# NVIDIA-Merlin/distributed-embeddings

Hardware: NVIDIA H100
Metric: DLRM global samples/sec (device-timed, max over ranks) (higher is better)
Workload: dtype bf16

## Files before the change

distributed_embeddings_b200/models/dlrm_fast.py:

```python
from __future__ import annotations

import os
from typing import Optional

import torch
from torch import nn

from ..ops import _native
from ..parallel.comm import CommContext
from ..parallel.fused import FusedEngine
from ..utils import nvtx
from ..utils.lr_schedule import LearningRateScheduler
from .dlrm import DLRM


def _pad8(n: int) -> int:
  return (n + 7) // 8 * 8


class _Layer:

  def __init__(self, lin: nn.Linear, relu: bool):
    self.lin = lin
    self.relu = relu
# ... 75 lines not shown
      dp_targets = []
      for layer, (off, shape) in zip(self.emb.dp_layers, self._dp_slots):
        n = shape[0] * shape[1]
        view = self.p32[off:off + n].view(shape)
        view.copy_(layer.embeddings.data)
        layer.embeddings.data = view
        dp_targets.append(self.g32[off:off + n].view(shape))
      if self._dp_slots:
        self.engine.set_dp_grad_targets(dp_targets)
        self.engine._tables_dirty = True
        self.engine._key = None
      for L in layers:
        wv = self.p32[L.w_off:L.w_off + L.w_numel].view(L.out_f, L.in_pad)
        wv[:, :L.in_f].copy_(L.lin.weight)
        L.lin.weight.data = wv[:, :L.in_f]
        bv = self.p32[L.b_off:L.b_off + L.out_f]
        bv.copy_(L.lin.bias)
        L.lin.bias.data = bv
        L.w16 = self.p16[L.w_off:L.w_off + L.w_numel].view(L.out_f, L.in_pad)
        L.b16 = self.p16[L.b_off:L.b_off + L.out_f]
        L.gw = self.g32[L.w_off:L.w_off + L.w_numel].view(L.out_f, L.in_pad)
        L.gb = self.g32[L.b_off:L.b_off + L.b_numel]
        L.w16T = torch.empty(L.in_pad, L.out_f, dtype=torch.bfloat16, device=dev)
      self.p16.copy_(self.p32)
      self._refresh_transposes()
    self.lr_t = torch.full((1,), float(lr), dtype=torch.float32, device=dev)
    self.engine.share_lr(self.lr_t)
    self.lr = float(lr)
    self.loss = torch.zeros(1, dtype=torch.float32, device=dev)
    self._batch = None
    self._graph = None
    self._side = torch.cuda.Stream(device=dev) if overlap else None
    self._wgrad_overlap = os.environ.get("DE_B200_WGRAD_STREAM", "auto")
    self._wstream = torch.cuda.Stream(device=dev) if overlap else None
    ar_env = os.environ.get("DE_B200_AR_OVERLAP", "auto")
    ar_on = ar_env == "1" or (ar_env == "auto" and self.world >= 4)
    self._ar_stream = torch.cuda.Stream(device=dev) if (overlap and self.world > 1 and ar_on) \
        else None

  def _refresh_transposes(self):
    if self.gemm == "cublas":
      return
    for L in self.bottom[1:] + self.top[1:]:
      L.w16T.copy_(L.w16.t())

  def _linear_fwd(self, L, x):
    if self.gemm in ("tcgen05", "tcgen05_pair"):
      pair = self.gemm == "tcgen05_pair" and L.out_f >= 256
      self.ops.gemm_tn_bias_act(x, L.w16, L.b16, L.y, True, 512 if pair else 0)
    else:
      torch._addmm_activation(L.b16, x, L.w16.t(), out=L.y)
    return L.y

  def _wgrad(self, L, x):
    use = self._wstream is not None and (
        self._wgrad_overlap == "1" or
        (self._wgrad_overlap == "auto" and (self._batch or 0) >= 49152))
    if not use:
      torch.mm(L.dy.t(), x, out_dtype=torch.float32, out=L.gw)
      return
    self._w_used = True
    self._wstream.wait_stream(torch.cuda.current_stream())
    with torch.cuda.stream(self._wstream):
      torch.mm(L.dy.t(), x, out_dtype=torch.float32, out=L.gw)

  def _dgrad_relu(self, L, x_below, dx, gb_below):
    if self.gemm == "cublas":
      torch.mm(L.dy, L.w16, out=dx)
      self.ops.relu_bwd_bias(dx, x_below, gb_below)
    else:
      self.ops.gemm_dgrad_relu_bias(L.dy, L.w16T, x_below, dx, gb_below, 0)

  def _alloc(self, b: int):
    dev, bf = self.dev, torch.bfloat16
    if self._stream_push:
      self.engine.enable_streamed_push(max(1024, -(-b // 16)))
    self.engine.prepare(b, [1] * self.n_emb, ids64=False)
    self.cat_stage = self.engine.in_flat[:self.n_emb * b].view(self.n_emb, b)
    self.num_in = torch.zeros(b, self.bottom[0].in_f, dtype=torch.float32, device=dev)
    self.lab_in = torch.zeros(b, dtype=torch.float32, device=dev)
    self.x0 = torch.zeros(b, self.bottom[0].in_pad, dtype=bf, device=dev)
    for L in self.bottom + self.top:
      L.y = torch.empty(b, L.out_f, dtype=bf, device=dev)
      L.dy = torch.empty(b, L.out_f, dtype=bf, device=dev)
    self.z = torch.zeros(b, self.top[0].in_pad, dtype=bf, device=dev)
    self.dz = torch.empty(b, self.top[0].in_pad, dtype=bf, device=dev)
    self._batch = b
    self._graph = None
    self._stage = [(torch.zeros_like(self.cat_stage), torch.zeros_like(self.num_in),
                    torch.zeros_like(self.lab_in)) for _ in range(2)]
    self._slot_dev = torch.zeros(1, dtype=torch.int32, device=dev)
    self._slot_host = torch.tensor([[0], [1]], dtype=torch.int32).pin_memory()
    self._h2d_done = [torch.cuda.Event(), torch.cuda.Event()]
    self._consumed = [torch.cuda.Event(), torch.cuda.Event()]
# ... 41 lines not shown
      L = self.top[i]
      x = self.top[i - 1].y if i > 0 else self.z
      dx = self.top[i - 1].dy if i > 0 else self.dz
      self._wgrad(L, x)
      if i > 0:
        self._dgrad_relu(L, x, dx, self.top[i - 1].gb)
      else:
        torch.mm(L.dy, L.w16, out=dx)
    if self._ar_stream is not None:
      ar = self._ar_stream
      ar.wait_stream(torch.cuda.current_stream())
      if getattr(self, "_w_used", False):
        ar.wait_stream(self._wstream)
      off = self.top[0].w_off
      with torch.cuda.stream(ar):
        self.ctx.allreduce_(self.gsym, self.n_flat - off, torch.float32, scale=1.0 / self.world,
                            byte_offset=off * 4, max_blocks=32)
    hb = self.bottom[-1]
    pushed = eng.streamed_push
    if pushed:
      eng.push_counters.zero_()
      self._push_ready.record(torch.cuda.current_stream())
      ops.interact_bwd(hb.y, eng.out, self.n_emb, self.dz, hb.dy, 0, 0, 1.0, eng.routes_stage,
                       len(eng.routes_stage_np), [], eng.push_counters, eng.push_chunk_rows)
      self._push_stream.wait_event(self._push_ready)
      with torch.cuda.stream(self._push_stream):
        eng.launch_streamed_push()
    else:
      ops.interact_bwd(hb.y, eng.out, self.n_emb, self.dz, hb.dy, 0, 0, 1.0, eng.routes_all,
                       len(eng.routes_all_np), eng.sync_grad_signal(), None, 0)
    if self._side is not None:
      self._side.wait_stream(torch.cuda.current_stream())
      if pushed:
        self._side.wait_stream(self._push_stream)
      with torch.cuda.stream(self._side):
        eng.backward_inplace()
    else:
      if pushed:
        torch.cuda.current_stream().wait_stream(self._push_stream)
      eng.backward_inplace()
    ops.relu_bwd_bias(hb.dy, hb.y, hb.gb)
    for i in range(len(self.bottom) - 1, -1, -1):
      L = self.bottom[i]
      x = self.bottom[i - 1].y if i > 0 else self.x0
      self._wgrad(L, x)
      if i > 0:
        self._dgrad_relu(L, x, self.bottom[i - 1].dy, self.bottom[i - 1].gb)
    if self._dp_slots and self._side is not None:
      torch.cuda.current_stream().wait_stream(self._side)
    if getattr(self, "_w_used", False):
      torch.cuda.current_stream().wait_stream(self._wstream)
      self._w_used = False
    if self.world > 1:
      if self._ar_stream is not None:
        ar = self._ar_stream
        ar.wait_stream(torch.cuda.current_stream())
        with torch.cuda.stream(ar):
          self.ctx.allreduce_(self.gsym, self.top[0].w_off, torch.float32, scale=1.0 / self.world)
        torch.cuda.current_stream().wait_stream(ar)
      else:
        self.ctx.allreduce_(self.gsym, self.n_flat, torch.float32, scale=1.0 / self.world)
    ops.dense_sgd(self.p32, self.p16, self.g32, self.lr_t, 1.0)
    self._refresh_transposes()
    if self._side is not None:
# ... 86 lines not shown
```

distributed_embeddings_b200/ops/csrc/bindings.cpp:

```cpp
#include <ATen/cuda/CUDAContext.h>
#include <c10/cuda/CUDAGuard.h>
#include <c10/cuda/CUDAStream.h>
#include <cuda_runtime.h>
#include <torch/library.h>
#include <torch/torch.h>

#include <cstdlib>
#include <cstring>
#include <mutex>
#include <string>
#include <unordered_map>
#include <vector>

#include "de_b200.h"

namespace {

using at::Tensor;

#define DE_CUDA_CHECK(expr)                                                              \
  do {                                                                                   \
    cudaError_t _e = (expr);                                                             \
    TORCH_CHECK(_e == cudaSuccess, "CUDA error in " #expr ": ", cudaGetErrorString(_e)); \
  } while (0)
// ... 696 lines not shown
}

void interact_fwd(const Tensor& bottom, const Tensor& emb, int64_t n_emb, Tensor z,
                  at::IntArrayRef sync) {
  check_bf16_2d(bottom, "bottom");
  check_bf16_2d(emb, "emb");
  check_bf16_2d(z, "z");
  c10::cuda::CUDAGuard guard(bottom.device());
  const int64_t dim = bottom.size(1);
  TORCH_CHECK(emb.size(1) == n_emb * dim);
  const int64_t need = (n_emb + 1) * n_emb / 2 + dim;
  TORCH_CHECK(z.size(1) >= need, "z is too narrow");
  bool ok = de::launch_interact_fwd(bottom.data_ptr(), bottom.stride(0), emb.data_ptr(),
                                    emb.stride(0), static_cast<int>(n_emb), static_cast<int>(dim),
                                    z.data_ptr(), z.stride(0), static_cast<int>(z.size(1)),
                                    bottom.size(0), sm_count(), cur_stream(), to_sync(sync));
  TORCH_CHECK(ok, "unsupported interaction shape (n_emb <= 31, dim in {16,32,64,128})");
  check_launch();
}

void interact_bwd(const Tensor& bottom, const Tensor& emb, int64_t n_emb, const Tensor& dz,
                  Tensor dbottom, int64_t demb_ptr, int64_t demb_stride, double emb_grad_scale,
                  const c10::optional<Tensor>& routes, int64_t n_routes, at::IntArrayRef sync,
                  const c10::optional<Tensor>& done_counters, int64_t chunk_rows) {
  check_bf16_2d(bottom, "bottom");
  check_bf16_2d(emb, "emb");
  check_bf16_2d(dz, "dz");
  check_bf16_2d(dbottom, "dbottom");
  if (routes.has_value())
    TORCH_CHECK(routes->is_cuda() && routes->scalar_type() == at::kByte &&
                routes->numel() >= n_routes * static_cast<int64_t>(sizeof(de::GradRoute)));
  c10::cuda::CUDAGuard guard(bottom.device());
  const int64_t dim = bottom.size(1);
  bool ok = de::launch_interact_bwd(bottom.data_ptr(), bottom.stride(0), emb.data_ptr(),
                                    emb.stride(0), static_cast<int>(n_emb), static_cast<int>(dim),
                                    dz.data_ptr(), dz.stride(0), dbottom.data_ptr(),
                                    dbottom.stride(0), reinterpret_cast<void*>(demb_ptr),
                                    demb_stride, static_cast<float>(emb_grad_scale),
                                    bottom.size(0), sm_count(), cur_stream(),
                                    routes.has_value()
                                        ? reinterpret_cast<const de::GradRoute*>(routes->data_ptr())
                                        : nullptr,
                                    static_cast<int>(n_routes), to_sync(sync),
                                    done_counters.has_value()
                                        ? reinterpret_cast<uint32_t*>(done_counters->data_ptr<int>())
                                        : nullptr,
                                    static_cast<int>(chunk_rows));
  TORCH_CHECK(ok, "unsupported interaction shape (n_emb <= 31, dim in {32,64,128}; routed / "
                  "signalling launches need dim in {64,128} and 16-byte aligned rows)");
  check_launch();
}

void avgpool_fwd(const Tensor& x, int64_t n, Tensor out, int64_t stride) {
  check_bf16_2d(x, "x");
  check_bf16_2d(out, "out");
  const int64_t out_len = (n + stride - 1) / stride;
  TORCH_CHECK(x.size(1) >= n && out.size(1) >= out_len && out.size(0) == x.size(0));
  const int64_t pad = std::max<int64_t>(0, (out_len - 1) * stride + stride - n);
  c10::cuda::CUDAGuard guard(x.device());
  de::launch_avgpool_fwd(x.data_ptr(), x.stride(0), static_cast<int>(n), out.data_ptr(),
                         out.stride(0), static_cast<int>(out_len), static_cast<int>(stride),
                         static_cast<int>(pad / 2), x.size(0), cur_stream());
  check_launch();
}

void avgpool_bwd(const Tensor& dout, Tensor dx, int64_t n, int64_t stride) {
  check_bf16_2d(dout, "dout");
  check_bf16_2d(dx, "dx");
  const int64_t out_len = (n + stride - 1) / stride;
  TORCH_CHECK(dx.size(1) >= n && dout.size(1) >= out_len && dout.size(0) == dx.size(0));
// ... 221 lines not shown
      "-> ()",
      &push_grad);
  m.def(
      "stream_push(int[] src_ptrs, int[] dst_ptrs, int[] row_bytes, Tensor counters, "
      "int chunk_rows, int rows, int blocks, int[] sync) -> ()",
      &stream_push);
  m.def(
      "rowslice_reduce(Tensor partial, int out_ptr, int out_stride, int out_dtype, Tensor cols) "
      "-> ()",
      &rowslice_reduce);
  m.def(
      "gather_ragged(Tensor segs, int[] val_ptrs, int[] split_ptrs, Tensor(a!) dst_vals, "
      "Tensor(b!) goff, int b, int max_cap) -> ()",
      &gather_ragged);
  m.def("select_copy(Tensor[] src0, Tensor[] src1, Tensor(a!)[] dst, Tensor slot_flag) -> ()",
        &select_copy);
  m.def("copy_cast_2d(Tensor src, int dst_ptr, int dst_stride, int dst_dtype, float scale) -> ()",
        &copy_cast_2d);
  m.def("interact_fwd(Tensor bottom, Tensor emb, int n_emb, Tensor(a!) z, int[] sync) -> ()",
        &interact_fwd);
  m.def(
      "interact_bwd(Tensor bottom, Tensor emb, int n_emb, Tensor dz, Tensor(a!) dbottom, "
      "int demb_ptr, int demb_stride, float emb_grad_scale, Tensor? routes, int n_routes, "
      "int[] sync, Tensor? done_counters, int chunk_rows) -> ()",
      &interact_bwd);
  m.def("avgpool_fwd(Tensor x, int n, Tensor(a!) out, int stride) -> ()", &avgpool_fwd);
  m.def("avgpool_bwd(Tensor dout, Tensor(a!) dx, int n, int stride) -> ()", &avgpool_bwd);
  m.def("relu_bwd_bias(Tensor(a!) dy, Tensor y, Tensor(b!) db) -> ()", &relu_bwd_bias);
  m.def(
      "head_loss(Tensor x, Tensor w, Tensor bias, Tensor labels, float inv_batch, Tensor(a!) dx, "
      "Tensor(b!) dw, Tensor(c!) db, Tensor(d!) dbias_prev, Tensor(e!) loss_sum, Tensor? logits) "
      "-> ()",
      &head_loss);
  m.def(
      "dense_sgd(Tensor(a!) p32, Tensor(b!) p16, Tensor(c!) g32, Tensor lr, float grad_scale) "
      "-> ()",
      &dense_sgd);
  m.def("cast_pad(Tensor src, Tensor(a!) dst) -> ()", &cast_pad);
  m.def(
      "gemm_tn_bias_act(Tensor a, Tensor b, Tensor? bias, Tensor(a!) out, bool relu, int block_n) "
      "-> ()",
      &gemm_tn_bias_act);
  m.def(
      "gemm_dgrad_relu_bias(Tensor dy, Tensor wt, Tensor act, Tensor(a!) dx, Tensor(b!) colsum, "
      "int block_n) -> ()",
      &gemm_dgrad_relu_bias);
  m.def("symm_alloc(int nbytes, int device_index) -> Tensor", &symm_alloc);
// ... 6 lines not shown
```

distributed_embeddings_b200/ops/csrc/de_b200.h:

```cpp
#pragma once
#include <cuda_runtime.h>
#include <stdint.h>

namespace de {

constexpr int kMaxPeers = 16;
constexpr int kGridCapSms = 132;

struct alignas(16) InputDesc {
  const void* table;
  const void* ids;
  const int64_t* offsets;
  int64_t ids_off;
  int64_t id_shift;
  int64_t sub_rows;
  int64_t row_base;
  int32_t width;
  int32_t hotness;
  int32_t dst_col;
  int32_t combiner;
  int32_t local_table;
  int32_t flags;
  int64_t item_off;
};
// ... 144 lines not shown
                            int n_cols, cudaStream_t stream);
void launch_gather_segments(const int64_t* segs, int n_seg, const PeerPtrs& src, void* dst,
                            int elem_bytes, int64_t max_seg_elems, cudaStream_t stream);
void launch_gather_ragged(const int64_t* segs, int n_seg, const PeerPtrs& src_vals,
                          const PeerPtrs& src_splits, void* dst_vals, int64_t* goff, int64_t b,
                          int world, int elem_bytes, int64_t max_cap, cudaStream_t stream);
void launch_select_copy(const void* const* src0, const void* const* src1, void* const* dst,
                        const int64_t* nbytes, int count, const int* slot_flag, int sm_count,
                        cudaStream_t stream);
void launch_copy_cast_2d(const void* src, int64_t src_stride, void* dst, int64_t dst_stride,
                         int64_t rows, int64_t cols, int src_dtype, int dst_dtype, float scale,
                         cudaStream_t stream);

bool launch_interact_fwd(const void* bottom, int64_t bottom_stride, const void* emb,
                         int64_t emb_stride, int n_emb, int dim, void* z, int64_t z_stride,
                         int z_width, int64_t batch, int sm_count, cudaStream_t stream,
                         const SyncArgs& sync);
bool launch_interact_bwd(const void* bottom, int64_t bottom_stride, const void* emb,
                         int64_t emb_stride, int n_emb, int dim, const void* dz,
                         int64_t dz_stride, void* dbottom, int64_t dbottom_stride, void* demb,
                         int64_t demb_stride, float emb_grad_scale, int64_t batch, int sm_count,
                         cudaStream_t stream, const GradRoute* routes, int n_routes,
                         const SyncArgs& sync, uint32_t* done_counters = nullptr,
                         int chunk_rows = 0);
void launch_avgpool_fwd(const void* x, int64_t x_stride, int n, void* out, int64_t out_stride,
                        int out_len, int stride, int left, int64_t rows, cudaStream_t stream);
void launch_avgpool_bwd(const void* dout, int64_t dout_stride, int out_len, void* dx,
                        int64_t dx_stride, int n, int stride, int left, int64_t rows,
                        cudaStream_t stream);
void launch_relu_bwd_bias(void* dy, const void* y, float* db, int64_t rows, int cols,
                          cudaStream_t stream);
bool launch_head_loss(const void* x, int K, const void* w, const void* bias, const float* labels,
                      int64_t batch, float inv_batch, void* dx, float* dw, float* db,
                      float* dbias_prev, float* loss_sum, float* logits_out, int sm_count,
                      cudaStream_t stream);
void launch_sgd_update(float* p32, void* p16, float* g32, const float* lr_ptr, float grad_scale,
                       int64_t n, int sm_count, cudaStream_t stream);
void launch_cast_pad(const float* src, int src_cols, void* dst, int dst_cols, int64_t rows,
                     cudaStream_t stream);

bool launch_gemm_tn_fused(const void* A, int64_t lda, const void* B, int64_t ldb, const void* bias,
                          void* C, int64_t ldc, int M, int N, int K, int epi, const void* act,
                          int64_t ldact, float* colsum, int block_n, int sm_count,
                          cudaStream_t stream);
bool launch_gemm_tn_bias_act(const void* A, int64_t lda, const void* B, int64_t ldb,
                             const void* bias, void* C, int64_t ldc, int M, int N, int K,
                             bool relu, int block_n, int sm_count, cudaStream_t stream);
// ... 3 lines not shown
```

distributed_embeddings_b200/ops/csrc/dense_kernels.cu:

```cuda
#include <cuda_bf16.h>
#include <cuda_runtime.h>
#include <stdint.h>

#include <cstdlib>

#include "common.cuh"
#include "de_b200.h"

namespace de {

namespace {

using bf16 = __nv_bfloat16;

__device__ __forceinline__ uint32_t smem_u32(const void* p) {
  return static_cast<uint32_t>(__cvta_generic_to_shared(p));
}

__device__ __forceinline__ void ldmatrix_x4(uint32_t (&r)[4], uint32_t addr) {
  asm volatile("ldmatrix.sync.aligned.m8n8.x4.shared.b16 {%0,%1,%2,%3}, [%4];"
               : "=r"(r[0]), "=r"(r[1]), "=r"(r[2]), "=r"(r[3])
               : "r"(addr));
}
__device__ __forceinline__ void ldmatrix_x4_trans(uint32_t (&r)[4], uint32_t addr) {
// ... 226 lines not shown
#pragma unroll 4
  for (int c = lane; c < total; c += 32) {
    const int row = c / kChunks, ch = c - row * kChunks;
    const bf16* src = row == 0 ? bottom + ch * 8 : emb + (row - 1) * D + ch * 8;
    cp_async16(sF + row * LD + ch * 8, src);
  }
  for (int c = lane; c < dz_chunks; c += 32) cp_async16(sDz + c * 8, dz + c * 8);
}

struct ChunkDst {
  unsigned long long base;
  long long stride;
};

template <int D>
__global__ void __launch_bounds__(kWarps * 32)
interact_bwd_v2_kernel(const bf16* __restrict__ bottom, int64_t bottom_stride,
                       const bf16* __restrict__ emb, int64_t emb_stride, int n_emb,
                       const bf16* __restrict__ dz, int64_t dz_stride, bf16* __restrict__ dbottom,
                       int64_t dbottom_stride, bf16* __restrict__ demb, int64_t demb_stride,
                       float emb_grad_scale, int64_t batch,
                       const GradRoute* __restrict__ routes, int n_routes,
                       const __grid_constant__ SyncArgs sync, uint32_t* __restrict__ done_counters,
                       int chunk_rows) {
  constexpr int LD = D + 8;
  constexpr int LDG = 40;
  constexpr int kWarpElems = 2 * kMaxFeat * LD + 2 * kDzMax + kMaxFeat * LDG;
  constexpr int kRowChunks = D / 8;
  extern __shared__ __align__(16) unsigned char smem_raw[];
  const int warp = threadIdx.x >> 5, lane = threadIdx.x & 31;
  bf16* base = reinterpret_cast<bf16*>(smem_raw) + warp * kWarpElems;
  bf16* sDz0 = base + 2 * kMaxFeat * LD;
  bf16* sG = sDz0 + 2 * kDzMax;
  ChunkDst* sDst = reinterpret_cast<ChunkDst*>(reinterpret_cast<bf16*>(smem_raw) +
                                               kWarps * kWarpElems);
  const int nf = n_emb + 1;
  const int n_inter = nf * (nf - 1) / 2;
  const int dz_chunks = (n_inter + D + 7) >> 3;
  const int n_chunks = n_emb * kRowChunks;
  if (routes == nullptr) {
    for (int c = threadIdx.x; c < n_chunks; c += blockDim.x) {
      sDst[c].base = reinterpret_cast<unsigned long long>(demb + c * 8);
      sDst[c].stride = demb_stride * 2;
    }
  } else {
    for (int r = 0; r < n_routes; ++r) {
      const GradRoute R = routes[r];
      const int c0 = R.src_col >> 3, nc = R.width >> 3;
      for (int c = threadIdx.x; c < nc; c += blockDim.x) {
        sDst[c0 + c].base =
            reinterpret_cast<unsigned long long>(reinterpret_cast<bf16*>(R.dst) + R.dst_col + c * 8);
        sDst[c0 + c].stride = R.dst_stride * 2;
      }
    }
  }
  zero_pad_rows<D>(base, LD, n_emb, lane);
  zero_pad_rows<D>(base + kMaxFeat * LD, LD, n_emb, lane);
  __syncthreads();

  const int64_t stride = static_cast<int64_t>(gridDim.x) * kWarps;
  int64_t s = static_cast<int64_t>(blockIdx.x) * kWarps + warp;
  int cur = 0;
// ... 43 lines not shown
        const int ncol = n0 + ((lane >> 4) << 3);
        ldmatrix_x4_trans(b01, smem_u32(sF + krow * LD + ncol));
        ldmatrix_x4_trans(b23, smem_u32(sF + krow * LD + ncol + 16));
#pragma unroll
        for (int mt = 0; mt < 2; ++mt) {
          mma_bf16(acc[mt][0], ga[mt][ks], b01[0], b01[1]);
          mma_bf16(acc[mt][1], ga[mt][ks], b01[2], b01[3]);
          mma_bf16(acc[mt][2], ga[mt][ks], b23[0], b23[1]);
          mma_bf16(acc[mt][3], ga[mt][ks], b23[2], b23[3]);
        }
      }
#pragma unroll
      for (int mt = 0; mt < 2; ++mt) {
#pragma unroll
        for (int nt = 0; nt < 4; ++nt) {
#pragma unroll
          for (int half = 0; half < 2; ++half) {
            const int row = mt * 16 + cr + half * 8;
            const int col = n0 + nt * 8 + cc;
            float v0 = acc[mt][nt][half * 2], v1 = acc[mt][nt][half * 2 + 1];
            if (row == 0) {
              v0 += __bfloat162float(sDz[n_inter + col]);
              v1 += __bfloat162float(sDz[n_inter + col + 1]);
            } else {
              v0 *= emb_grad_scale;
              v1 *= emb_grad_scale;
            }
            if (row <= n_emb)
              *reinterpret_cast<__nv_bfloat162*>(sF + row * LD + col) =
                  __floats2bfloat162_rn(v0, v1);
          }
        }
      }
    }
    __syncwarp();
    if (lane < kRowChunks)
      *reinterpret_cast<uint4*>(dbottom + s * dbottom_stride + lane * 8) =
          *reinterpret_cast<const uint4*>(sF + lane * 8);
    for (int c = lane; c < n_chunks; c += 32) {
      const int row = 1 + c / kRowChunks, ch = c - (row - 1) * kRowChunks;
      const ChunkDst d = sDst[c];
      *reinterpret_cast<uint4*>(d.base + static_cast<unsigned long long>(s * d.stride)) =
          *reinterpret_cast<const uint4*>(sF + row * LD + ch * 8);
    }
    __syncwarp();
    if (done_counters != nullptr && lane == 0) {
      __threadfence();
      atomicAdd(done_counters + s / chunk_rows, 1u);
    }
  }
  cp_async_wait_group<0>();
  sync_tail(sync);
}

constexpr int kRbUnroll = 4;
__global__ void __launch_bounds__(256)
relu_bwd_bias_kernel(bf16* __restrict__ dy, const bf16* __restrict__ y, float* __restrict__ db,
                     int64_t rows, int cols, int rows_per_block) {
  extern __shared__ float s_part[];
  const int tpr = cols >> 3;
  const int rows_par = blockDim.x / tpr;
  const int tr = threadIdx.x / tpr, tc = threadIdx.x - tr * tpr;
  const int64_t r0 = static_cast<int64_t>(blockIdx.x) * rows_per_block;
  const int64_t r1 = min(rows, r0 + rows_per_block);
  float acc[8] = {0, 0, 0, 0, 0, 0, 0, 0};
  if (tr < rows_par) {
    for (int64_t r = r0 + tr; r < r1; r += static_cast<int64_t>(rows_par) * kRbUnroll) {
      uint4 g[kRbUnroll], a[kRbUnroll];
#pragma unroll
      for (int u = 0; u < kRbUnroll; ++u) {
        const int64_t rr = r + static_cast<int64_t>(u) * rows_par;
        if (rr < r1) {
          g[u] = *reinterpret_cast<const uint4*>(dy + rr * cols + tc * 8);
          a[u] = *reinterpret_cast<const uint4*>(y + rr * cols + tc * 8);
        }
      }
#pragma unroll
      for (int u = 0; u < kRbUnroll; ++u) {
        const int64_t rr = r + static_cast<int64_t>(u) * rows_par;
        if (rr < r1) {
          uint32_t* gw = reinterpret_cast<uint32_t*>(&g[u]);
          const uint32_t* aw = reinterpret_cast<const uint32_t*>(&a[u]);
#pragma unroll
          for (int i = 0; i < 4; ++i) {
            float2 gf = __bfloat1622float2(*reinterpret_cast<__nv_bfloat162*>(&gw[i]));
            const float2 af = __bfloat1622float2(*reinterpret_cast<const __nv_bfloat162*>(&aw[i]));
            gf.x = af.x > 0.f ? gf.x : 0.f;
            gf.y = af.y > 0.f ? gf.y : 0.f;
            acc[2 * i] += gf.x;
            acc[2 * i + 1] += gf.y;
            __nv_bfloat162 h = __floats2bfloat162_rn(gf.x, gf.y);
            gw[i] = *reinterpret_cast<uint32_t*>(&h);
          }
          *reinterpret_cast<uint4*>(dy + rr * cols + tc * 8) = g[u];
        }
      }
    }
#pragma unroll
    for (int i = 0; i < 8; ++i) s_part[tr * cols + tc * 8 + i] = acc[i];
  }
  __syncthreads();
  for (int c = threadIdx.x; c < cols; c += blockDim.x) {
    float v = 0.f;
    for (int t = 0; t < rows_par; ++t) v += s_part[t * cols + c];
    atomicAdd(db + c, v);
  }
}

template <int PL>
__global__ void __launch_bounds__(256)
head_loss_kernel(const bf16* __restrict__ x, int K, const bf16* __restrict__ w,
                 const bf16* __restrict__ bias, const float* __restrict__ labels, int64_t batch,
                 float inv_batch, bf16* __restrict__ dx, float* __restrict__ dw,
                 float* __restrict__ db, float* __restrict__ dbias_prev,
                 float* __restrict__ loss_sum, float* __restrict__ logits_out) {
  extern __shared__ float sred[];
  float* s_dw = sred;
// ... 170 lines not shown
#define DE_IFWD(DD)                                                                              \
  {                                                                                              \
    const size_t smem = kWarps * fwd_warp_bytes(DD);                                             \
    cudaFuncSetAttribute(interact_fwd_kernel<DD>, cudaFuncAttributeMaxDynamicSharedMemorySize,   \
                         static_cast<int>(smem));                                                \
    interact_fwd_kernel<DD><<<static_cast<unsigned>(blocks), kWarps * 32, smem, stream>>>(       \
        reinterpret_cast<const bf16*>(bottom), bottom_stride, reinterpret_cast<const bf16*>(emb), \
        emb_stride, n_emb, reinterpret_cast<bf16*>(z), z_stride, z_width, batch, sync);          \
    return true;                                                                                 \
  }
  if (dim == 128) DE_IFWD(128)
  if (dim == 64) DE_IFWD(64)
  if (dim == 32) DE_IFWD(32)
  if (dim == 16) DE_IFWD(16)
#undef DE_IFWD
  return false;
}

bool launch_interact_bwd(const void* bottom, int64_t bottom_stride, const void* emb,
                         int64_t emb_stride, int n_emb, int dim, const void* dz,
                         int64_t dz_stride, void* dbottom, int64_t dbottom_stride, void* demb,
                         int64_t demb_stride, float emb_grad_scale, int64_t batch, int sm_count,
                         cudaStream_t stream, const GradRoute* routes, int n_routes,
                         const SyncArgs& sync, uint32_t* done_counters, int chunk_rows) {
  if (n_emb + 1 > kMaxFeat || batch <= 0 || dim % 32 != 0) return false;
  int64_t blocks = (batch + kWarps - 1) / kWarps;
  const int64_t cap = static_cast<int64_t>(sm_count) * 8;
  if (blocks > cap) blocks = cap;
  static const bool force_v1 = [] {
    const char* v = std::getenv("DE_B200_INTERACT_V1");
    return v != nullptr && v[0] == '1';
  }();
  const int nf = n_emb + 1;
  const int dz_elems = (nf * (nf - 1) / 2 + dim + 7) / 8 * 8;
  const bool v2_ok =
      dz_elems <= kDzMax && dz_elems <= dz_stride && dz_stride % 8 == 0 &&
      bottom_stride % 8 == 0 && emb_stride % 8 == 0 && dbottom_stride % 8 == 0 &&
      ((reinterpret_cast<uintptr_t>(dz) | reinterpret_cast<uintptr_t>(bottom) |
        reinterpret_cast<uintptr_t>(emb) | reinterpret_cast<uintptr_t>(dbottom)) & 15) == 0 &&
      (dim == 128 || dim == 64) &&
      (routes != nullptr || (demb_stride % 8 == 0 && (reinterpret_cast<uintptr_t>(demb) & 15) == 0));
  if ((routes != nullptr || done_counters != nullptr) && !v2_ok) return false;
  const bool has_sync = sync.state != nullptr && (sync.wait_ch >= 0 || sync.signal_ch >= 0);
  if (v2_ok && (!force_v1 || routes != nullptr || has_sync || done_counters != nullptr)) {
    int64_t blocks2 = (batch + kWarps - 1) / kWarps;
    if (blocks2 > static_cast<int64_t>(sm_count) * 2) blocks2 = static_cast<int64_t>(sm_count) * 2;
#define DE_IBWD2(DD)                                                                             \
  {                                                                                              \
    const size_t smem =                                                                          \
        kWarps * (2 * kMaxFeat * (DD + 8) + 2 * kDzMax + kMaxFeat * 40) * sizeof(bf16) +         \
        static_cast<size_t>(n_emb) * (DD / 8) * sizeof(ChunkDst);                                \
    cudaFuncSetAttribute(interact_bwd_v2_kernel<DD>,                                             \
                         cudaFuncAttributeMaxDynamicSharedMemorySize, static_cast<int>(smem));   \
    interact_bwd_v2_kernel<DD><<<static_cast<unsigned>(blocks2), kWarps * 32, smem, stream>>>(   \
        reinterpret_cast<const bf16*>(bottom), bottom_stride, reinterpret_cast<const bf16*>(emb), \
        emb_stride, n_emb, reinterpret_cast<const bf16*>(dz), dz_stride,                         \
        reinterpret_cast<bf16*>(dbottom), dbottom_stride, reinterpret_cast<bf16*>(demb),         \
        demb_stride, emb_grad_scale, batch, routes, n_routes, sync, done_counters, chunk_rows);  \
    return true;                                                                                 \
  }
    if (dim == 128) DE_IBWD2(128)
    if (dim == 64) DE_IBWD2(64)
#undef DE_IBWD2
  }
  if (has_sync) return false;
#define DE_IBWD(DD)                                                                              \
  {                                                                                              \
    const size_t smem = kWarps * (kMaxFeat * (DD + 8) + kMaxFeat * 40) * sizeof(bf16);           \
    cudaFuncSetAttribute(interact_bwd_kernel<DD>, cudaFuncAttributeMaxDynamicSharedMemorySize,   \
                         static_cast<int>(smem));                                                \
    interact_bwd_kernel<DD><<<static_cast<unsigned>(blocks), kWarps * 32, smem, stream>>>(       \
        reinterpret_cast<const bf16*>(bottom), bottom_stride, reinterpret_cast<const bf16*>(emb), \
        emb_stride, n_emb, reinterpret_cast<const bf16*>(dz), dz_stride,                         \
        reinterpret_cast<bf16*>(dbottom), dbottom_stride, reinterpret_cast<bf16*>(demb),         \
        demb_stride, emb_grad_scale, batch);                                                     \
    return true;                                                                                 \
  }
  if (dim == 128) DE_IBWD(128)
  if (dim == 64) DE_IBWD(64)
  if (dim == 32) DE_IBWD(32)
#undef DE_IBWD
  return false;
}

void launch_relu_bwd_bias(void* dy, const void* y, float* db, int64_t rows, int cols,
                          cudaStream_t stream) {
  if (rows <= 0) return;
  const int tpr = cols / 8;
  const int threads = 256;
  const int rows_par = threads / tpr;
  const int rows_per_block = rows_par * kRbUnroll * 4;
  const int64_t blocks = (rows + rows_per_block - 1) / rows_per_block;
  const size_t smem = static_cast<size_t>(rows_par) * cols * sizeof(float);
  relu_bwd_bias_kernel<<<static_cast<unsigned>(blocks), threads, smem, stream>>>(
      reinterpret_cast<bf16*>(dy), reinterpret_cast<const bf16*>(y), db, rows, cols,
      rows_per_block);
}

bool launch_head_loss(const void* x, int K, const void* w, const void* bias, const float* labels,
                      int64_t batch, float inv_batch, void* dx, float* dw, float* db,
                      float* dbias_prev, float* loss_sum, float* logits_out, int sm_count,
                      cudaStream_t stream) {
  if (batch <= 0) return true;
  const int threads = 256;
  int64_t blocks = (batch + 7) / 8;
  if (blocks > sm_count * 4) blocks = sm_count * 4;
  const size_t smem = (2 * K + 2) * sizeof(float);
#define DE_HEAD(PL)                                                                              \
  head_loss_kernel<PL><<<static_cast<unsigned>(blocks), threads, smem, stream>>>(                \
      reinterpret_cast<const bf16*>(x), K, reinterpret_cast<const bf16*>(w),                     \
      reinterpret_cast<const bf16*>(bias), labels, batch, inv_batch, reinterpret_cast<bf16*>(dx), \
      dw, db, dbias_prev, loss_sum, logits_out)
  switch (K) {
    case 64: DE_HEAD(2); break;
    case 128: DE_HEAD(4); break;
    case 256: DE_HEAD(8); break;
    case 512: DE_HEAD(16); break;
    case 1024: DE_HEAD(32); break;
    default: return false;
// ... 26 lines not shown
```

distributed_embeddings_b200/ops/csrc/gemm_wgmma.cu:

```cuda
#include <cuda.h>
#include <cuda_bf16.h>
#include <cuda_runtime.h>
#include <stdint.h>

#include <mutex>

#include "de_b200.h"

namespace de {

namespace {

using bf16 = __nv_bfloat16;

constexpr int BLOCK_M = 128;
constexpr int BLOCK_K = 64;
constexpr int WGMMA_N = 128;
constexpr int WGMMA_K = 16;
constexpr int kGemmThreads = 384;
constexpr int kMaxColsum = 2048;

__device__ __forceinline__ uint32_t smem_addr(const void* p) {
  return static_cast<uint32_t>(__cvta_generic_to_shared(p));
}
// ... 299 lines not shown
    float acc[BLOCK_N / WGMMA_N][64];
#pragma unroll
    for (int nb = 0; nb < BLOCK_N / WGMMA_N; ++nb)
#pragma unroll
      for (int r = 0; r < 64; ++r) acc[nb][r] = 0.f;
    int stage = 0;
    uint32_t phase = 0;
    for (int tile = blockIdx.x; tile < num_tiles; tile += gridDim.x) {
      const int m0 = (tile / tiles_n) * BLOCK_M, n0 = (tile % tiles_n) * BLOCK_N;
      consumer_tile<BLOCK_N, STAGES, EPI, false>(smem, full_bar, empty_bar, stage, phase, m0, n0,
                                                 num_kb, cw, bias, C, ldc, M, N, act, ldact,
                                                 s_colsum, acc);
    }
    if (EPI == 2) {
      consumer_bar_sync();
      for (int i = threadIdx.x - 128; i < N && i < kMaxColsum; i += 256) {
        const float vsum = s_colsum[i];
        if (vsum != 0.f) atomicAdd(colsum + i, vsum);
      }
    }
  }
}

__device__ __forceinline__ uint32_t cluster_ctarank() {
  uint32_t r;
  asm volatile("mov.u32 %0, %%cluster_ctarank;" : "=r"(r));
  return r;
}
__device__ __forceinline__ void cluster_sync_all() {
  asm volatile("barrier.cluster.arrive.release.aligned;" ::: "memory");
  asm volatile("barrier.cluster.wait.acquire.aligned;" ::: "memory");
}

template <int BLOCK_N, int STAGES, int EPI>
__global__ void __cluster_dims__(2, 1, 1) __launch_bounds__(kGemmThreads, 1)
gemm_tn_pair_kernel(const __grid_constant__ CUtensorMap tma_a,
                    const __grid_constant__ CUtensorMap tma_b, const bf16* __restrict__ bias,
                    bf16* __restrict__ C, int64_t ldc, int M, int N, int K) {
  using L = SmemLayout<BLOCK_N, STAGES>;
  constexpr int kHalfB = L::kBBytes / 2;
  extern __shared__ uint8_t smem_raw[];
  uint8_t* smem = reinterpret_cast<uint8_t*>(
      (reinterpret_cast<uintptr_t>(smem_raw) + 1023) & ~static_cast<uintptr_t>(1023));
  uint64_t* full_bar = reinterpret_cast<uint64_t*>(smem + L::kBarOffset);
  uint64_t* empty_bar = full_bar + STAGES;

// ... 118 lines not shown
    return launch_one<BLOCK_N, STAGES, 0>(ta, tb, bias, C, ldc, M, N, K, act, ldact, colsum,
                                          sm_count, stream);
  if (epi == 1)
    return launch_one<BLOCK_N, STAGES, 1>(ta, tb, bias, C, ldc, M, N, K, act, ldact, colsum,
                                          sm_count, stream);
  return launch_one<BLOCK_N, STAGES, 2>(ta, tb, bias, C, ldc, M, N, K, act, ldact, colsum,
                                        sm_count, stream);
}

}

bool launch_gemm_tn_fused(const void* A, int64_t lda, const void* B, int64_t ldb, const void* bias,
                          void* C, int64_t ldc, int M, int N, int K, int epi, const void* act,
                          int64_t ldact, float* colsum, int block_n, int sm_count,
                          cudaStream_t stream) {
  if (M <= 0 || N <= 0 || K <= 0) return true;
  if ((lda % 8) || (ldb % 8) || (ldc % 8) || (N % 8)) return false;
  if ((reinterpret_cast<uintptr_t>(A) | reinterpret_cast<uintptr_t>(B) |
       reinterpret_cast<uintptr_t>(C)) & 15)
    return false;
  if (epi == 2 && (act == nullptr || colsum == nullptr || N > kMaxColsum || (ldact % 8) ||
                   (reinterpret_cast<uintptr_t>(act) & 15)))
    return false;
  const int bn = (block_n == 128 || block_n == 256) ? block_n : (N >= 256 ? 256 : 128);
  alignas(64) CUtensorMap ta, tb;
  if (!make_tensor_map(&ta, A, M, K, lda, BLOCK_M)) return false;
  if (!make_tensor_map(&tb, B, N, K, ldb, bn)) return false;
  if (bn == 256)
    return launch_cfg<256, 4>(ta, tb, bias, C, ldc, M, N, K, epi, act, ldact, colsum, sm_count,
                              stream);
  return launch_cfg<128, 6>(ta, tb, bias, C, ldc, M, N, K, epi, act, ldact, colsum, sm_count,
                            stream);
}

namespace {
template <int EPI>
bool launch_pair(const CUtensorMap& ta, const CUtensorMap& tb, const void* bias, void* C,
                 int64_t ldc, int M, int N, int K, int sm_count, cudaStream_t stream) {
  constexpr int BN = 256, ST = 4;
  using L = SmemLayout<BN, ST>;
  const size_t smem = L::kTotal + 1024;
  const int tiles = ((N + BN - 1) / BN) * ((M + 2 * BLOCK_M - 1) / (2 * BLOCK_M));
  int pairs = sm_count / 2;
  if (tiles < pairs) pairs = tiles;
  if (pairs < 1) return false;
  cudaFuncSetAttribute(gemm_tn_pair_kernel<BN, ST, EPI>,
                       cudaFuncAttributeMaxDynamicSharedMemorySize, static_cast<int>(smem));
  gemm_tn_pair_kernel<BN, ST, EPI><<<dim3(2 * pairs), kGemmThreads, smem, stream>>>(
// ... 31 lines not shown
```

Before: 14.86 million.

## Fuse ReLU-bias backward into interaction bwd and add ping-pong dgrad GEMM

Makes the fused dgrad+ReLU+bias-grad GEMM path apply whenever shapes allow, even in cuBLAS mode, replacing a separate mm plus relu_bwd_bias pass. Adds a new warp-specialized ping-pong WGMMA dgrad kernel with TMA activation loads and TMA stores for the epi==2, block_n==0 case. Also folds the top bottom-MLP layer's ReLU mask and bias-gradient reduction into the interaction backward kernel, which drops one elementwise pass over the activations. This adds shared-memory atomics and extra smem use in interaction bwd, and the new GEMM kernel may be slower than cuBLAS for some shapes.

```diff
diff --git a/distributed_embeddings_b200/models/dlrm_fast.py b/distributed_embeddings_b200/models/dlrm_fast.py
--- a/distributed_embeddings_b200/models/dlrm_fast.py
+++ b/distributed_embeddings_b200/models/dlrm_fast.py
@@ -121,6 +121,7 @@
         L.gw = self.g32[L.w_off:L.w_off + L.w_numel].view(L.out_f, L.in_pad)
         L.gb = self.g32[L.b_off:L.b_off + L.b_numel]
         L.w16T = torch.empty(L.in_pad, L.out_f, dtype=torch.bfloat16, device=dev)
+        L.fused_dgrad = L.in_f <= 2048 and L.in_f % 8 == 0 and L.out_f % 8 == 0
       self.p16.copy_(self.p32)
       self._refresh_transposes()
     self.lr_t = torch.full((1,), float(lr), dtype=torch.float32, device=dev)
@@ -138,8 +139,6 @@
         else None
 
   def _refresh_transposes(self):
-    if self.gemm == "cublas":
-      return
     for L in self.bottom[1:] + self.top[1:]:
       L.w16T.copy_(L.w16.t())
 
@@ -164,11 +163,11 @@
       torch.mm(L.dy.t(), x, out_dtype=torch.float32, out=L.gw)
 
   def _dgrad_relu(self, L, x_below, dx, gb_below):
-    if self.gemm == "cublas":
+    if L.fused_dgrad:
+      self.ops.gemm_dgrad_relu_bias(L.dy, L.w16T, x_below, dx, gb_below, 0)
+    else:
       torch.mm(L.dy, L.w16, out=dx)
       self.ops.relu_bwd_bias(dx, x_below, gb_below)
-    else:
-      self.ops.gemm_dgrad_relu_bias(L.dy, L.w16T, x_below, dx, gb_below, 0)
 
   def _alloc(self, b: int):
     dev, bf = self.dev, torch.bfloat16
@@ -256,13 +255,13 @@
       eng.push_counters.zero_()
       self._push_ready.record(torch.cuda.current_stream())
       ops.interact_bwd(hb.y, eng.out, self.n_emb, self.dz, hb.dy, 0, 0, 1.0, eng.routes_stage,
-                       len(eng.routes_stage_np), [], eng.push_counters, eng.push_chunk_rows)
+                       len(eng.routes_stage_np), [], eng.push_counters, eng.push_chunk_rows, hb.gb)
       self._push_stream.wait_event(self._push_ready)
       with torch.cuda.stream(self._push_stream):
         eng.launch_streamed_push()
     else:
       ops.interact_bwd(hb.y, eng.out, self.n_emb, self.dz, hb.dy, 0, 0, 1.0, eng.routes_all,
-                       len(eng.routes_all_np), eng.sync_grad_signal(), None, 0)
+                       len(eng.routes_all_np), eng.sync_grad_signal(), None, 0, hb.gb)
     if self._side is not None:
       self._side.wait_stream(torch.cuda.current_stream())
       if pushed:
@@ -273,7 +272,6 @@
       if pushed:
         torch.cuda.current_stream().wait_stream(self._push_stream)
       eng.backward_inplace()
-    ops.relu_bwd_bias(hb.dy, hb.y, hb.gb)
     for i in range(len(self.bottom) - 1, -1, -1):
       L = self.bottom[i]
       x = self.bottom[i - 1].y if i > 0 else self.x0
diff --git a/distributed_embeddings_b200/ops/csrc/bindings.cpp b/distributed_embeddings_b200/ops/csrc/bindings.cpp
--- a/distributed_embeddings_b200/ops/csrc/bindings.cpp
+++ b/distributed_embeddings_b200/ops/csrc/bindings.cpp
@@ -742,7 +742,8 @@
 void interact_bwd(const Tensor& bottom, const Tensor& emb, int64_t n_emb, const Tensor& dz,
                   Tensor dbottom, int64_t demb_ptr, int64_t demb_stride, double emb_grad_scale,
                   const c10::optional<Tensor>& routes, int64_t n_routes, at::IntArrayRef sync,
-                  const c10::optional<Tensor>& done_counters, int64_t chunk_rows) {
+                  const c10::optional<Tensor>& done_counters, int64_t chunk_rows,
+                  const c10::optional<Tensor>& dbias) {
   check_bf16_2d(bottom, "bottom");
   check_bf16_2d(emb, "emb");
   check_bf16_2d(dz, "dz");
@@ -750,6 +751,9 @@
   if (routes.has_value())
     TORCH_CHECK(routes->is_cuda() && routes->scalar_type() == at::kByte &&
                 routes->numel() >= n_routes * static_cast<int64_t>(sizeof(de::GradRoute)));
+  if (dbias.has_value())
+    TORCH_CHECK(dbias->is_cuda() && dbias->scalar_type() == at::kFloat &&
+                dbias->numel() >= bottom.size(1));
   c10::cuda::CUDAGuard guard(bottom.device());
   const int64_t dim = bottom.size(1);
   bool ok = de::launch_interact_bwd(bottom.data_ptr(), bottom.stride(0), emb.data_ptr(),
@@ -765,7 +769,8 @@
                                     done_counters.has_value()
                                         ? reinterpret_cast<uint32_t*>(done_counters->data_ptr<int>())
                                         : nullptr,
-                                    static_cast<int>(chunk_rows));
+                                    static_cast<int>(chunk_rows),
+                                    dbias.has_value() ? dbias->data_ptr<float>() : nullptr);
   TORCH_CHECK(ok, "unsupported interaction shape (n_emb <= 31, dim in {32,64,128}; routed / "
                   "signalling launches need dim in {64,128} and 16-byte aligned rows)");
   check_launch();
@@ -1033,7 +1038,7 @@
   m.def(
       "interact_bwd(Tensor bottom, Tensor emb, int n_emb, Tensor dz, Tensor(a!) dbottom, "
       "int demb_ptr, int demb_stride, float emb_grad_scale, Tensor? routes, int n_routes, "
-      "int[] sync, Tensor? done_counters, int chunk_rows) -> ()",
+      "int[] sync, Tensor? done_counters, int chunk_rows, Tensor(b!)? dbias=None) -> ()",
       &interact_bwd);
   m.def("avgpool_fwd(Tensor x, int n, Tensor(a!) out, int stride) -> ()", &avgpool_fwd);
   m.def("avgpool_bwd(Tensor dout, Tensor(a!) dx, int n, int stride) -> ()", &avgpool_bwd);
diff --git a/distributed_embeddings_b200/ops/csrc/de_b200.h b/distributed_embeddings_b200/ops/csrc/de_b200.h
--- a/distributed_embeddings_b200/ops/csrc/de_b200.h
+++ b/distributed_embeddings_b200/ops/csrc/de_b200.h
@@ -190,7 +190,7 @@
                          int64_t demb_stride, float emb_grad_scale, int64_t batch, int sm_count,
                          cudaStream_t stream, const GradRoute* routes, int n_routes,
                          const SyncArgs& sync, uint32_t* done_counters = nullptr,
-                         int chunk_rows = 0);
+                         int chunk_rows = 0, float* dbias = nullptr);
 void launch_avgpool_fwd(const void* x, int64_t x_stride, int n, void* out, int64_t out_stride,
                         int out_len, int stride, int left, int64_t rows, cudaStream_t stream);
 void launch_avgpool_bwd(const void* dout, int64_t dout_stride, int out_len, void* dx,
diff --git a/distributed_embeddings_b200/ops/csrc/dense_kernels.cu b/distributed_embeddings_b200/ops/csrc/dense_kernels.cu
--- a/distributed_embeddings_b200/ops/csrc/dense_kernels.cu
+++ b/distributed_embeddings_b200/ops/csrc/dense_kernels.cu
@@ -272,7 +272,7 @@
                        float emb_grad_scale, int64_t batch,
                        const GradRoute* __restrict__ routes, int n_routes,
                        const __grid_constant__ SyncArgs sync, uint32_t* __restrict__ done_counters,
-                       int chunk_rows) {
+                       int chunk_rows, float* __restrict__ dbias) {
   constexpr int LD = D + 8;
   constexpr int LDG = 40;
   constexpr int kWarpElems = 2 * kMaxFeat * LD + 2 * kDzMax + kMaxFeat * LDG;
@@ -288,6 +288,9 @@
   const int n_inter = nf * (nf - 1) / 2;
   const int dz_chunks = (n_inter + D + 7) >> 3;
   const int n_chunks = n_emb * kRowChunks;
+  float* sDb = reinterpret_cast<float*>(sDst + n_chunks);
+  if (dbias != nullptr)
+    for (int c = threadIdx.x; c < kWarps * D; c += blockDim.x) sDb[c] = 0.f;
   if (routes == nullptr) {
     for (int c = threadIdx.x; c < n_chunks; c += blockDim.x) {
       sDst[c].base = reinterpret_cast<unsigned long long>(demb + c * 8);
@@ -377,6 +380,13 @@
             if (row == 0) {
               v0 += __bfloat162float(sDz[n_inter + col]);
               v1 += __bfloat162float(sDz[n_inter + col + 1]);
+              if (dbias != nullptr) {
+                const float2 y = __bfloat1622float2(*reinterpret_cast<const __nv_bfloat162*>(sF + col));
+                v0 = y.x > 0.f ? v0 : 0.f;
+                v1 = y.y > 0.f ? v1 : 0.f;
+                sDb[warp * D + col] += v0;
+                sDb[warp * D + col + 1] += v1;
+              }
             } else {
               v0 *= emb_grad_scale;
               v1 *= emb_grad_scale;
@@ -405,13 +415,22 @@
     }
   }
   cp_async_wait_group<0>();
+  if (dbias != nullptr) {
+    __syncthreads();
+    for (int c = threadIdx.x; c < D; c += blockDim.x) {
+      float v = 0.f;
+#pragma unroll
+      for (int w = 0; w < kWarps; ++w) v += sDb[w * D + c];
+      if (v != 0.f) atomicAdd(dbias + c, v);
+    }
+  }
   sync_tail(sync);
 }
 
 constexpr int kRbUnroll = 4;
 __global__ void __launch_bounds__(256)
 relu_bwd_bias_kernel(bf16* __restrict__ dy, const bf16* __restrict__ y, float* __restrict__ db,
-                     int64_t rows, int cols, int rows_per_block) {
+                     int64_t rows, int cols, int64_t ld, int rows_per_block) {
   extern __shared__ float s_part[];
   const int tpr = cols >> 3;
   const int rows_par = blockDim.x / tpr;
@@ -426,8 +445,8 @@
       for (int u = 0; u < kRbUnroll; ++u) {
         const int64_t rr = r + static_cast<int64_t>(u) * rows_par;
         if (rr < r1) {
-          g[u] = *reinterpret_cast<const uint4*>(dy + rr * cols + tc * 8);
-          a[u] = *reinterpret_cast<const uint4*>(y + rr * cols + tc * 8);
+          g[u] = *reinterpret_cast<const uint4*>(dy + rr * ld + tc * 8);
+          a[u] = *reinterpret_cast<const uint4*>(y + rr * ld + tc * 8);
         }
       }
 #pragma unroll
@@ -447,7 +466,7 @@
             __nv_bfloat162 h = __floats2bfloat162_rn(gf.x, gf.y);
             gw[i] = *reinterpret_cast<uint32_t*>(&h);
           }
-          *reinterpret_cast<uint4*>(dy + rr * cols + tc * 8) = g[u];
+          *reinterpret_cast<uint4*>(dy + rr * ld + tc * 8) = g[u];
         }
       }
     }
@@ -664,7 +683,8 @@
                          int64_t dz_stride, void* dbottom, int64_t dbottom_stride, void* demb,
                          int64_t demb_stride, float emb_grad_scale, int64_t batch, int sm_count,
                          cudaStream_t stream, const GradRoute* routes, int n_routes,
-                         const SyncArgs& sync, uint32_t* done_counters, int chunk_rows) {
+                         const SyncArgs& sync, uint32_t* done_counters, int chunk_rows,
+                         float* dbias) {
   if (n_emb + 1 > kMaxFeat || batch <= 0 || dim % 32 != 0) return false;
   int64_t blocks = (batch + kWarps - 1) / kWarps;
   const int64_t cap = static_cast<int64_t>(sm_count) * 8;
@@ -691,14 +711,16 @@
   {                                                                                              \
     const size_t smem =                                                                          \
         kWarps * (2 * kMaxFeat * (DD + 8) + 2 * kDzMax + kMaxFeat * 40) * sizeof(bf16) +         \
-        static_cast<size_t>(n_emb) * (DD / 8) * sizeof(ChunkDst);                                \
+        static_cast<size_t>(n_emb) * (DD / 8) * sizeof(ChunkDst) +                               \
+        (dbias != nullptr ? kWarps * DD * sizeof(float) : 0);                                    \
     cudaFuncSetAttribute(interact_bwd_v2_kernel<DD>,                                             \
                          cudaFuncAttributeMaxDynamicSharedMemorySize, static_cast<int>(smem));   \
     interact_bwd_v2_kernel<DD><<<static_cast<unsigned>(blocks2), kWarps * 32, smem, stream>>>(   \
         reinterpret_cast<const bf16*>(bottom), bottom_stride, reinterpret_cast<const bf16*>(emb), \
         emb_stride, n_emb, reinterpret_cast<const bf16*>(dz), dz_stride,                         \
         reinterpret_cast<bf16*>(dbottom), dbottom_stride, reinterpret_cast<bf16*>(demb),         \
-        demb_stride, emb_grad_scale, batch, routes, n_routes, sync, done_counters, chunk_rows);  \
+        demb_stride, emb_grad_scale, batch, routes, n_routes, sync, done_counters, chunk_rows,   \
+        dbias);                                                                                  \
     return true;                                                                                 \
   }
     if (dim == 128) DE_IBWD2(128)
@@ -706,6 +728,7 @@
 #undef DE_IBWD2
   }
   if (has_sync) return false;
+  if (dbias != nullptr && (bottom_stride != dim || dbottom_stride != dim)) return false;
 #define DE_IBWD(DD)                                                                              \
   {                                                                                              \
     const size_t smem = kWarps * (kMaxFeat * (DD + 8) + kMaxFeat * 40) * sizeof(bf16);           \
@@ -716,6 +739,7 @@
         emb_stride, n_emb, reinterpret_cast<const bf16*>(dz), dz_stride,                         \
         reinterpret_cast<bf16*>(dbottom), dbottom_stride, reinterpret_cast<bf16*>(demb),         \
         demb_stride, emb_grad_scale, batch);                                                     \
+    if (dbias != nullptr) launch_relu_bwd_bias(dbottom, bottom, dbias, batch, DD, stream);       \
     return true;                                                                                 \
   }
   if (dim == 128) DE_IBWD(128)
@@ -728,15 +752,18 @@
 void launch_relu_bwd_bias(void* dy, const void* y, float* db, int64_t rows, int cols,
                           cudaStream_t stream) {
   if (rows <= 0) return;
-  const int tpr = cols / 8;
   const int threads = 256;
-  const int rows_par = threads / tpr;
-  const int rows_per_block = rows_par * kRbUnroll * 4;
-  const int64_t blocks = (rows + rows_per_block - 1) / rows_per_block;
-  const size_t smem = static_cast<size_t>(rows_par) * cols * sizeof(float);
-  relu_bwd_bias_kernel<<<static_cast<unsigned>(blocks), threads, smem, stream>>>(
-      reinterpret_cast<bf16*>(dy), reinterpret_cast<const bf16*>(y), db, rows, cols,
-      rows_per_block);
+  for (int c0 = 0; c0 < cols; c0 += threads * 8) {
+    const int w = cols - c0 < threads * 8 ? cols - c0 : threads * 8;
+    const int tpr = w / 8;
+    const int rows_par = threads / tpr;
+    const int rows_per_block = rows_par * kRbUnroll * 4;
+    const int64_t blocks = (rows + rows_per_block - 1) / rows_per_block;
+    const size_t smem = static_cast<size_t>(rows_par) * w * sizeof(float);
+    relu_bwd_bias_kernel<<<static_cast<unsigned>(blocks), threads, smem, stream>>>(
+        reinterpret_cast<bf16*>(dy) + c0, reinterpret_cast<const bf16*>(y) + c0, db + c0, rows, w,
+        cols, rows_per_block);
+  }
 }
 
 bool launch_head_loss(const void* x, int K, const void* w, const void* bias, const float* labels,
diff --git a/distributed_embeddings_b200/ops/csrc/gemm_wgmma.cu b/distributed_embeddings_b200/ops/csrc/gemm_wgmma.cu
--- a/distributed_embeddings_b200/ops/csrc/gemm_wgmma.cu
+++ b/distributed_embeddings_b200/ops/csrc/gemm_wgmma.cu
@@ -345,6 +345,198 @@
   }
 }
 
+__device__ __forceinline__ void named_bar_sync(int id, int count) {
+  asm volatile("bar.sync %0, %1;" ::"r"(id), "r"(count) : "memory");
+}
+__device__ __forceinline__ void named_bar_arrive(int id, int count) {
+  asm volatile("bar.arrive %0, %1;" ::"r"(id), "r"(count) : "memory");
+}
+__device__ __forceinline__ void tma_store_2d(const CUtensorMap* map, const void* smem_src, int c0,
+                                             int c1) {
+  asm volatile(
+      "cp.async.bulk.tensor.2d.global.shared::cta.bulk_group [%0, {%2, %3}], [%1];" ::"l"(map),
+      "r"(smem_addr(smem_src)), "r"(c0), "r"(c1)
+      : "memory");
+}
+__device__ __forceinline__ void tma_store_commit() {
+  asm volatile("cp.async.bulk.commit_group;" ::: "memory");
+}
+template <int N>
+__device__ __forceinline__ void tma_store_wait_read() {
+  asm volatile("cp.async.bulk.wait_group.read %0;" ::"n"(N) : "memory");
+}
+template <int N>
+__device__ __forceinline__ void tma_store_wait_all() {
+  asm volatile("cp.async.bulk.wait_group %0;" ::"n"(N) : "memory");
+}
+
+constexpr int kPpBlockN = 128;
+constexpr int kPpStages = 4;
+constexpr int kPpTileBytes = BLOCK_M * kPpBlockN * 2;
+
+struct PingPongLayout {
+  using Ring = SmemLayout<kPpBlockN, kPpStages>;
+  static constexpr int kStagingOffset = kPpStages * Ring::kStageBytes;
+  static constexpr int kColsumOffset = kStagingOffset + 2 * kPpTileBytes;
+  static constexpr int kBarOffset = kColsumOffset + kMaxColsum * 4;
+  static constexpr int kNumBars = 2 * kPpStages + 4;
+  static constexpr int kTotal = kBarOffset + kNumBars * 8;
+};
+
+__global__ void __launch_bounds__(kGemmThreads, 1)
+gemm_dgrad_pingpong_kernel(const __grid_constant__ CUtensorMap tma_a,
+                           const __grid_constant__ CUtensorMap tma_b,
+                           const __grid_constant__ CUtensorMap tma_act,
+                           const __grid_constant__ CUtensorMap tma_c, int M, int N, int K,
+                           float* __restrict__ colsum) {
+  using L = PingPongLayout;
+  using R = L::Ring;
+  extern __shared__ uint8_t smem_raw[];
+  uint8_t* smem = reinterpret_cast<uint8_t*>(
+      (reinterpret_cast<uintptr_t>(smem_raw) + 1023) & ~static_cast<uintptr_t>(1023));
+  float* s_colsum = reinterpret_cast<float*>(smem + L::kColsumOffset);
+  uint64_t* full_bar = reinterpret_cast<uint64_t*>(smem + L::kBarOffset);
+  uint64_t* empty_bar = full_bar + kPpStages;
+  uint64_t* act_full = empty_bar + kPpStages;
+  uint64_t* staging_empty = act_full + 2;
+
+  const int wg = threadIdx.x >> 7;
+  const int num_kb = (K + BLOCK_K - 1) / BLOCK_K;
+  const int tiles_n = (N + kPpBlockN - 1) / kPpBlockN;
+  const int num_tiles = tiles_n * ((M + BLOCK_M - 1) / BLOCK_M);
+  const int my_tiles =
+      num_tiles > static_cast<int>(blockIdx.x)
+          ? (num_tiles - static_cast<int>(blockIdx.x) + gridDim.x - 1) / gridDim.x
+          : 0;
+
+  if (threadIdx.x == 0) {
+    tma_prefetch_desc(&tma_a);
+    tma_prefetch_desc(&tma_b);
+    tma_prefetch_desc(&tma_act);
+    tma_prefetch_desc(&tma_c);
+    for (int s = 0; s < kPpStages; ++s) {
+      mbar_init(&full_bar[s], 1);
+      mbar_init(&empty_bar[s], 1);
+    }
+    for (int c = 0; c < 2; ++c) {
+      mbar_init(&act_full[c], 1);
+      mbar_init(&staging_empty[c], 1);
+    }
+    fence_barrier_init();
+    fence_proxy_async();
+  }
+  for (int i = threadIdx.x; i < kMaxColsum; i += kGemmThreads) s_colsum[i] = 0.f;
+  __syncthreads();
+
+  if (wg == 0) {
+    asm volatile("setmaxnreg.dec.sync.aligned.u32 40;");
+    if (threadIdx.x == 0) {
+      int it = 0;
+      for (int j = 0; j < my_tiles; ++j) {
+        const int tile = blockIdx.x + j * gridDim.x;
+        const int m0 = (tile / tiles_n) * BLOCK_M, n0 = (tile % tiles_n) * kPpBlockN;
+        for (int kb = 0; kb < num_kb; ++kb, ++it) {
+          const int stage = it % kPpStages;
+          mbar_wait(&empty_bar[stage], ((it / kPpStages) & 1) ^ 1);
+          uint8_t* sa = smem + stage * R::kStageBytes;
+          mbar_expect_tx(&full_bar[stage], R::kStageBytes);
+          tma_load_2d(sa, &tma_a, &full_bar[stage], kb * BLOCK_K, m0);
+          tma_load_2d(sa + R::kABytes, &tma_b, &full_bar[stage], kb * BLOCK_K, n0);
+        }
+        const int c = j & 1;
+        uint8_t* st = smem + L::kStagingOffset + c * kPpTileBytes;
+        mbar_wait(&staging_empty[c], ((j >> 1) & 1) ^ 1);
+        mbar_expect_tx(&act_full[c], kPpTileBytes);
+        tma_load_2d(st, &tma_act, &act_full[c], n0, m0);
+        tma_load_2d(st + kPpTileBytes / 2, &tma_act, &act_full[c], n0 + 64, m0);
+      }
+    }
+  } else {
+    asm volatile("setmaxnreg.inc.sync.aligned.u32 232;");
+    const int cw = wg - 1;
+    const int lane = threadIdx.x & 31, warp_in_wg = (threadIdx.x >> 5) & 3;
+    const bool leader = warp_in_wg == 0 && lane == 0;
+    uint8_t* st = smem + L::kStagingOffset + cw * kPpTileBytes;
+    float acc[2][64];
+    for (int j = cw; j < my_tiles; j += 2) {
+      const int tile = blockIdx.x + j * gridDim.x;
+      const int m0 = (tile / tiles_n) * BLOCK_M, n0 = (tile % tiles_n) * kPpBlockN;
+      if (j > 0) named_bar_sync(2 + cw, 256);
+      int it = j * num_kb, prev_stage = -1;
+      for (int kb = 0; kb < num_kb; ++kb, ++it) {
+        const int stage = it % kPpStages;
+        mbar_wait(&full_bar[stage], (it / kPpStages) & 1);
+        const uint32_t sa = smem_addr(smem + stage * R::kStageBytes);
+        const uint32_t sb = sa + R::kABytes;
+        wgmma_fence();
+#pragma unroll
+        for (int k = 0; k < BLOCK_K / WGMMA_K; ++k) {
+          const uint64_t db = make_sw128_kmajor_desc(sb + k * WGMMA_K * 2);
+#pragma unroll
+          for (int h = 0; h < 2; ++h)
+            wgmma_m64n128k16(acc[h], make_sw128_kmajor_desc(sa + h * 64 * 128 + k * WGMMA_K * 2),
+                             db, (kb | k) != 0 ? 1u : 0u);
+        }
+        wgmma_commit();
+        wgmma_wait<1>();
+        if (prev_stage >= 0 && leader) mbar_arrive(&empty_bar[prev_stage]);
+        prev_stage = stage;
+      }
+      wgmma_wait<0>();
+      if (prev_stage >= 0 && leader) mbar_arrive(&empty_bar[prev_stage]);
+      if (j + 1 < my_tiles) named_bar_arrive(2 + (cw ^ 1), 256);
+
+      mbar_wait(&act_full[cw], (j >> 1) & 1);
+      const int rbase = warp_in_wg * 16 + (lane >> 2);
+#pragma unroll
+      for (int q = 0; q < kPpBlockN / 8; ++q) {
+        const int col = n0 + q * 8 + (lane & 3) * 2;
+        uint8_t* chunk_base = st + (q >> 3) * (kPpTileBytes / 2) +
+                              ((((q & 7) ^ (lane >> 2))) << 4) + (lane & 3) * 4;
+        float cs0 = 0.f, cs1 = 0.f;
+#pragma unroll
+        for (int h = 0; h < 2; ++h) {
+#pragma unroll
+          for (int i = 0; i < 2; ++i) {
+            __nv_bfloat162* p =
+                reinterpret_cast<__nv_bfloat162*>(chunk_base + (h * 64 + rbase + 8 * i) * 128);
+            const float2 af = __bfloat1622float2(*p);
+            const float v0 = af.x > 0.f ? acc[h][4 * q + 2 * i] : 0.f;
+            const float v1 = af.y > 0.f ? acc[h][4 * q + 2 * i + 1] : 0.f;
+            cs0 += v0;
+            cs1 += v1;
+            *p = __floats2bfloat162_rn(v0, v1);
+          }
+        }
+#pragma unroll
+        for (int sft = 4; sft < 32; sft <<= 1) {
+          cs0 += __shfl_xor_sync(0xffffffffu, cs0, sft);
+          cs1 += __shfl_xor_sync(0xffffffffu, cs1, sft);
+        }
+        if (lane < 4 && col < N) {
+          atomicAdd(&s_colsum[col], cs0);
+          atomicAdd(&s_colsum[col + 1], cs1);
+        }
+      }
+      fence_proxy_async();
+      named_bar_sync(4 + cw, 128);
+      if (leader) {
+        tma_store_2d(&tma_c, st, n0, m0);
+        tma_store_2d(&tma_c, st + kPpTileBytes / 2, n0 + 64, m0);
+        tma_store_commit();
+        tma_store_wait_read<0>();
+        mbar_arrive(&staging_empty[cw]);
+      }
+    }
+    if (leader) tma_store_wait_all<0>();
+    consumer_bar_sync();
+    for (int i = threadIdx.x - 128; i < N && i < kMaxColsum; i += 256) {
+      const float vsum = s_colsum[i];
+      if (vsum != 0.f) atomicAdd(colsum + i, vsum);
+    }
+  }
+}
+
 __device__ __forceinline__ uint32_t cluster_ctarank() {
   uint32_t r;
   asm volatile("mov.u32 %0, %%cluster_ctarank;" : "=r"(r));
@@ -509,8 +701,25 @@
   if (epi == 2 && (act == nullptr || colsum == nullptr || N > kMaxColsum || (ldact % 8) ||
                    (reinterpret_cast<uintptr_t>(act) & 15)))
     return false;
+  alignas(64) CUtensorMap ta, tb;
+  if (epi == 2 && block_n == 0) {
+    alignas(64) CUtensorMap tact, tc;
+    if (!make_tensor_map(&ta, A, M, K, lda, BLOCK_M) ||
+        !make_tensor_map(&tb, B, N, K, ldb, kPpBlockN) ||
+        !make_tensor_map(&tact, act, M, N, ldact, BLOCK_M) ||
+        !make_tensor_map(&tc, C, M, N, ldc, BLOCK_M))
+      return false;
+    using L = PingPongLayout;
+    const size_t smem = L::kTotal + 1024;
+    static_assert(L::kTotal + 1024 <= 227 * 1024, "exceeds the 227 KB of shared memory per block");
+    const int tiles = ((N + kPpBlockN - 1) / kPpBlockN) * ((M + BLOCK_M - 1) / BLOCK_M);
+    cudaFuncSetAttribute(gemm_dgrad_pingpong_kernel, cudaFuncAttributeMaxDynamicSharedMemorySize,
+                         static_cast<int>(smem));
+    gemm_dgrad_pingpong_kernel<<<dim3(tiles < sm_count ? tiles : sm_count), kGemmThreads, smem,
+                                 stream>>>(ta, tb, tact, tc, M, N, K, colsum);
+    return cudaGetLastError() == cudaSuccess;
+  }
   const int bn = (block_n == 128 || block_n == 256) ? block_n : (N >= 256 ? 256 : 128);
-  alignas(64) CUtensorMap ta, tb;
   if (!make_tensor_map(&ta, A, M, K, lda, BLOCK_M)) return false;
   if (!make_tensor_map(&tb, B, N, K, ldb, bn)) return false;
   if (bn == 256)
```

Result: slower. 14.65 million, median of 6 (-1.4%).
